# Antiparadox/Spartan-BN254

Hardware: AMD Instinct MI355X
Metric: msm_points_per_s (higher is better)
Workload: dtype u32; 1 GPU; synthetic BN254 G1 MSM, 2^20 uniform Fr scalars x distinct bases per GPU, inputs resident in HBM; steps_in_flight=6

## Files before the change

spartan-bn254_amd/csrc/glv_kernels.cuh:

```cuda
#pragma once
#include "msm_kernels.cuh"

namespace sbn {

namespace glv {
constexpr uint64_t A[2] = {0x8211bbeb7d4f1128ull, 0x6f4d8248eeb859fcull};
constexpr uint64_t B = 0x89d3256894d213e3ull;
constexpr uint64_t C[2] = {0x0be4e1541221250bull, 0x6f4d8248eeb859fdull};
constexpr uint64_t G1[3] = {0x5398fd0300ff6565ull, 0x4ccef014a773d2d2ull, 0x2ull};
constexpr uint64_t G2[2] = {0xd91d232ec7e0b3d7ull, 0x2ull};
constexpr uint64_t R[4] = {0x43e1f593f0000001ull, 0x2833e84879b97091ull, 0xb85045b68181585dull, 0x30644e72e131a029ull};
constexpr uint32_t BETA[8] = {0x607cfd48u, 0xe4bd44e5u, 0xbb966e3du, 0xc28f069fu, 0xe0acccb0u, 0x5e6dd9e7u, 0xe131a029u, 0x30644e72u};
}

template <int NA, int NB>
__device__ __forceinline__ void glv_mul(const uint64_t (&a)[NA], const uint64_t (&b)[NB], uint64_t (&out)[NA + NB]) {
#pragma unroll
  for (int i = 0; i < NA + NB; i++) out[i] = 0;
#pragma unroll
  for (int i = 0; i < NA; i++) {
    uint64_t carry = 0;
#pragma unroll
    for (int j = 0; j < NB; j++) {
      const uint64_t lo = a[i] * b[j], hi = __umul64hi(a[i], b[j]);
// ... 15 lines not shown
    for (int j = 0; j < NB && i + j < 4; j++) {
      const uint64_t lo = a[i] * b[j], hi = __umul64hi(a[i], b[j]);
      uint64_t s = out[i + j] + lo; uint64_t cy = s < lo ? 1 : 0;
      s += carry; cy += s < carry ? 1 : 0;
      out[i + j] = s; carry = hi + cy;
    }
    if (i + NB < 4) out[i + NB] = carry;
  }
}
__device__ __forceinline__ bool glv_diff_ge_r(const uint64_t (&x)[4], const uint64_t (&y)[4]) {
  uint64_t d[4], borrow = 0;
#pragma unroll
  for (int i = 0; i < 4; i++) { const uint64_t t = x[i] - y[i]; const uint64_t b1 = x[i] < y[i]; d[i] = t - borrow; borrow = b1 | (t < borrow); }
#pragma unroll
  for (int i = 3; i >= 0; i--) { if (d[i] != glv::R[i]) return d[i] > glv::R[i]; }
  return true;
}
__device__ __forceinline__ void u128_mul_lo(uint64_t a0, uint64_t a1, uint64_t b0, uint64_t b1, uint64_t& o0, uint64_t& o1) {
  o0 = a0 * b0; o1 = __umul64hi(a0, b0) + a0 * b1 + a1 * b0;
}
__device__ __forceinline__ void u128_add(uint64_t& x0, uint64_t& x1, uint64_t y0, uint64_t y1) { const uint64_t s = x0 + y0; x1 += y1 + (s < x0 ? 1 : 0); x0 = s; }
__device__ __forceinline__ void u128_sub(uint64_t& x0, uint64_t& x1, uint64_t y0, uint64_t y1) { const uint64_t b = x0 < y0 ? 1 : 0; x0 -= y0; x1 -= y1 + b; }

__device__ __forceinline__ void glv_split(const uint64_t (&k)[4], uint64_t (&k1)[2], uint64_t (&k2)[2]) {
  uint64_t p1[7], p2[6];
  glv_mul<4, 3>(k, glv::G1, p1);
  glv_mul<4, 2>(k, glv::G2, p2);
  uint64_t c1[2] = {p1[4], p1[5]}, c2[1] = {p2[4]};
  {
    uint64_t kc[4], cr[4];
    glv_mul_lo256<2>(k, glv::C, kc);
    const uint64_t c1v[4] = {c1[0], c1[1], 0, 0};
    glv_mul_lo256<4>(c1v, glv::R, cr);
    if (glv_diff_ge_r(kc, cr)) { if (++c1[0] == 0) ++c1[1]; }
  }
  {
    uint64_t kb[4], cr[4];
    const uint64_t bb[1] = {glv::B};
    glv_mul_lo256<1>(k, bb, kb);
    const uint64_t c2v[4] = {c2[0], 0, 0, 0};
    glv_mul_lo256<4>(c2v, glv::R, cr);
    if (glv_diff_ge_r(kb, cr)) ++c2[0];
  }
  uint64_t x0 = k[0], x1 = k[1], t0, t1;
  u128_mul_lo(c1[0], c1[1], glv::A[0], glv::A[1], t0, t1); u128_sub(x0, x1, t0, t1);
  u128_mul_lo(c2[0], 0, glv::B, 0, t0, t1); u128_sub(x0, x1, t0, t1);
  uint64_t y0, y1;
  u128_mul_lo(c1[0], c1[1], glv::B, 0, y0, y1);
  u128_mul_lo(c2[0], 0, glv::C[0], glv::C[1], t0, t1); u128_sub(y0, y1, t0, t1);
  if (y1 >> 63) { u128_add(x0, x1, glv::B, 0); u128_add(y0, y1, glv::C[0], glv::C[1]); }
  k1[0] = x0; k1[1] = x1; k2[0] = y0; k2[1] = y1;
}

__global__ void __launch_bounds__(256) k_glv_split(const uint32_t* __restrict__ scalars, size_t n, uint32_t* __restrict__ out, uint32_t* __restrict__ bad) {
  const size_t t = (size_t)blockIdx.x * blockDim.x + threadIdx.x;
  if (t >= n) return;
  const uint4 a = reinterpret_cast<const uint4*>(scalars + 8 * t)[0], b = reinterpret_cast<const uint4*>(scalars + 8 * t)[1];
  const uint32_t kk[8] = {a.x, a.y, a.z, a.w, b.x, b.y, b.z, b.w};
  uint64_t k1[2] = {0, 0}, k2[2] = {0, 0};
  if (!fe_is_canonical<FrP>(kk)) atomicAdd(bad, 1u);
  else {
    const uint64_t k[4] = {(uint64_t)a.x | ((uint64_t)a.y << 32), (uint64_t)a.z | ((uint64_t)a.w << 32), (uint64_t)b.x | ((uint64_t)b.y << 32), (uint64_t)b.z | ((uint64_t)b.w << 32)};
    glv_split(k, k1, k2);
  }
  uint4* o = reinterpret_cast<uint4*>(out);
  o[t] = make_uint4((uint32_t)k1[0], (uint32_t)(k1[0] >> 32), (uint32_t)k1[1], (uint32_t)(k1[1] >> 32));
  o[n + t] = make_uint4((uint32_t)k2[0], (uint32_t)(k2[0] >> 32), (uint32_t)k2[1], (uint32_t)(k2[1] >> 32));
}

__global__ void __launch_bounds__(256) k_glv_table(const uint32_t* __restrict__ pts, size_t npts, uint32_t* __restrict__ out) {
  const size_t j = (size_t)blockIdx.x * blockDim.x + threadIdx.x;
  if (j >= npts) return;
  const uint4* s = reinterpret_cast<const uint4*>(pts + 16 * j);
  uint4* d0 = reinterpret_cast<uint4*>(out + 16 * j);
  uint4* d1 = reinterpret_cast<uint4*>(out + 16 * (npts + j));
  const uint4 w0 = s[0], w1 = s[1], w2 = s[2], w3 = s[3];
  d0[0] = w0; d0[1] = w1; d0[2] = w2; d0[3] = w3;
  const Fq beta = fe_to_mont(fe_unpack<FqP>(glv::BETA));
  const Fq x = fe_load<FqP>(pts + 16 * j);
  fe_store<FqP>(out + 16 * (npts + j), fe_mul(x, beta));
  d1[2] = w2; d1[3] = w3;
}

}
```

spartan-bn254_amd/csrc/msm_host.hpp:

```cpp
#pragma once
static int ilog2_ceil(size_t n) { int l = 0; while (((size_t)1 << l) < n) l++; return l; }

static MsmShape make_shape(int c, int bits = 254) {
  MsmShape s; s.c = c; s.nb = 1 << (c - 1);
  int W = (bits + c - 1) / c;
  int tb = bits - (W - 1) * c;
  if (tb > c - 1) W += 1;
  s.W = W;
  return s;
}
static MsmShape choose_shape(size_t terms, bool shared_bucket_set, int cmax, size_t problems = 0, int chard = MSM_C_MAX) {
  const char* env = getenv("SBN_MSM_C");
  if (env && atoi(env) >= 7 && atoi(env) <= chard) return make_shape(atoi(env));
  if (cmax > chard) cmax = chard;
  if (problems && problems * terms <= 32768) {
    if (!shared_bucket_set && problems == 1 && terms >= 512 && terms <= 4096 && cmax >= 8) return make_shape(terms <= 512 ? 8 : 7);
    double bl = 1e300; int bcl = 7;
    for (int c = 7; c <= cmax; c++) {
      MsmShape s = make_shape(c);
      const int tb = 254 - (s.W - 1) * c;
      const double top = (double)terms / (double)(1u << (tb > 0 ? (tb < 20 ? tb : 20) : 0));
      const double load = (shared_bucket_set ? (double)terms * s.W / s.nb : (double)terms / s.nb) + top;
      if (load <= 6.0) return s;
      if (load < bl) { bl = load; bcl = c; }
    }
    return make_shape(bcl);
  }
  if (!shared_bucket_set && terms < ((size_t)1 << 20) && cmax >= 15) return make_shape(15);
  double best = 1e300; int bc = 7;
  for (int c = 7; c <= cmax; c++) {
    MsmShape s = make_shape(c);
    double sets = shared_bucket_set ? 1.0 : (double)s.W;
    const double per_bucket = (chard > MSM_C_MAX || (shared_bucket_set && problems >= 256)) ? 40.0 : 56.0;
    double cost = (double)terms * s.W * 10.0 + sets * s.nb * per_bucket;
    if (!shared_bucket_set && 254 - (s.W - 1) * c < c - 1) cost += (double)terms * 5.0;
    if (cost < best) { best = cost; bc = c; }
  }
  return make_shape(bc);
}

#define S2_FOR_EACH_C(X) X(13) X(14) X(15) X(16) X(17) X(18) X(19) X(20) X(21) X(22)
#define S2_GLV_FOR_EACH_C(X) X(13) X(14) X(15) X(16) X(17)
static bool sort2_set_lds() {
  bool ok = true;
  const int bytes = (int)s2_scatter_lds_bytes(S2_P_MAX);
  if (hipFuncSetAttribute((const void*)k_s2_place, hipFuncAttributeMaxDynamicSharedMemorySize, (int)s2_place_lds_bytes(S2_LO_LOG_MAX)) != hipSuccess) { (void)hipGetLastError(); ok = false; }
#define X(C) if (hipFuncSetAttribute((const void*)k_s2_scatter<C, S2_SPT>, hipFuncAttributeMaxDynamicSharedMemorySize, bytes) != hipSuccess) { (void)hipGetLastError(); ok = false; } \
             if (hipFuncSetAttribute((const void*)k_s2_scatter<C, S2_SPT_SMALL>, hipFuncAttributeMaxDynamicSharedMemorySize, bytes) != hipSuccess) { (void)hipGetLastError(); ok = false; }
  S2_FOR_EACH_C(X)
#undef X
  const int cnt_bytes = 24 * S2_P_MAX * 4;
#define X(C) if (hipFuncSetAttribute((const void*)k_s2_count<C, S2_SPT>, hipFuncAttributeMaxDynamicSharedMemorySize, cnt_bytes) != hipSuccess) { (void)hipGetLastError(); ok = false; } \
             if (hipFuncSetAttribute((const void*)k_s2_count<C, S2_SPT_SMALL>, hipFuncAttributeMaxDynamicSharedMemorySize, cnt_bytes) != hipSuccess) { (void)hipGetLastError(); ok = false; }
  S2_FOR_EACH_C(X)
#undef X
#define X(C) if (hipFuncSetAttribute((const void*)k_s2_count<C, S2_SPT, 4>, hipFuncAttributeMaxDynamicSharedMemorySize, cnt_bytes) != hipSuccess) { (void)hipGetLastError(); ok = false; } \
             if (hipFuncSetAttribute((const void*)k_s2_count<C, S2_SPT_SMALL, 4>, hipFuncAttributeMaxDynamicSharedMemorySize, cnt_bytes) != hipSuccess) { (void)hipGetLastError(); ok = false; } \
             if (hipFuncSetAttribute((const void*)k_s2_scatter<C, S2_SPT, 4>, hipFuncAttributeMaxDynamicSharedMemorySize, bytes) != hipSuccess) { (void)hipGetLastError(); ok = false; } \
             if (hipFuncSetAttribute((const void*)k_s2_scatter<C, S2_SPT_SMALL, 4>, hipFuncAttributeMaxDynamicSharedMemorySize, bytes) != hipSuccess) { (void)hipGetLastError(); ok = false; }
  S2_GLV_FOR_EACH_C(X)
#undef X
  return ok;
}
static bool sort2_applies(const sbn_ctx* c, int mode, size_t n, int cbits) {
  return mode == MODE_SINGLE && c->sort2_ok && c->sort2_min && n >= c->sort2_min && cbits >= S2_C_MIN && cbits <= S2_C_MAX;
}
static int sort2_run(sbn_ctx* c, const uint32_t* scalars, size_t n, const MsmShape& s, size_t estride, uint32_t* hist, uint32_t* offs, uint32_t* sorted, bool glv = false, size_t glv_gap = 0) {
  S2Geom g; g.n = n; g.c = s.c; g.W = s.W; g.half = n / 2; g.gap = glv ? glv_gap : 0;
  if (glv && (s.c < 13 || s.c > 17)) return fail(c, SBN_EINVAL, "two-level sort: no GLV instantiation for windows of %d bits", s.c);
  g.lo_log = std::max(s.c - 1 - 8, 8); if (g.lo_log > S2_LO_LOG_MAX) g.lo_log = S2_LO_LOG_MAX;
  if (const char* e = getenv("SBN_SORT2_LO")) { int v = atoi(e); if (v >= 4 && v <= S2_LO_LOG_MAX) g.lo_log = v; }
  if (s.c - 1 - g.lo_log < 0) g.lo_log = s.c - 1;
  while ((s.nb >> g.lo_log) > S2_P_MAX) g.lo_log++;
  if (g.lo_log > S2_LO_LOG_MAX) return fail(c, SBN_EINVAL, "two-level sort: window of %d bits is too wide", s.c);
  g.P = s.nb >> g.lo_log;
  const int LO = 1 << g.lo_log;
  int spt = (n <= ((size_t)1 << 21) && g.P <= 64) ? S2_SPT_SMALL : S2_SPT;
  if (const char* e = getenv("SBN_SORT2_SPT")) { const int v = atoi(e); if (v == S2_SPT || v == S2_SPT_SMALL) spt = v; }
  const size_t ch = (size_t)1024 * spt;
  g.K = (int)((n + ch - 1) / ch);
  const size_t WP = (size_t)g.W * g.P;
  const size_t max_sc = ((size_t)g.W * n) / S2_SUB + WP;
  int rc;
  if ((rc = ensure(c, c->s2_cnt, WP * g.K * 4))) return rc;
  if ((rc = ensure(c, c->s2_part, (3 * WP + 1) * 4))) return rc;
  if ((rc = ensure(c, c->s2_idx, (size_t)g.W * n * 4))) return rc;
  if ((rc = ensure(c, c->s2_lo, (size_t)g.W * n * 2))) return rc;
  if ((rc = ensure(c, c->blockhist, max_sc * LO * 4))) return rc;
  uint32_t* cntA = (uint32_t*)c->s2_cnt.p; uint32_t* part_cnt = (uint32_t*)c->s2_part.p; uint32_t* part_off = part_cnt + WP; uint32_t* sc_off = part_off + WP;
  uint32_t* tmp_idx = (uint32_t*)c->s2_idx.p; uint16_t* tmp_lo = (uint16_t*)c->s2_lo.p; uint32_t* bh = (uint32_t*)c->blockhist.p;
  const size_t lds_a = WP * 4, lds_c = s2_scatter_lds_bytes(g.P, spt);
  if (lds_a > (size_t)24 * S2_P_MAX * 4) return fail(c, SBN_EINVAL, "two-level sort: %zu level-1 counters do not fit the LDS granted to k_s2_count", WP);
  {
    ProfScope _ps(c, "k_s2_count");
    if (glv) switch (s.c) {
#define X(C) case C: if (spt == S2_SPT) hipLaunchKernelGGL((k_s2_count<C, S2_SPT, 4>), dim3(g.K), dim3(1024), lds_a, c->stream, scalars, g, cntA, c->d_bad); \
                     else hipLaunchKernelGGL((k_s2_count<C, S2_SPT_SMALL, 4>), dim3(g.K), dim3(1024), lds_a, c->stream, scalars, g, cntA, c->d_bad); break;
      S2_GLV_FOR_EACH_C(X)
#undef X
    } else switch (s.c) {
#define X(C) case C: if (spt == S2_SPT) hipLaunchKernelGGL((k_s2_count<C, S2_SPT>), dim3(g.K), dim3(1024), lds_a, c->stream, scalars, g, cntA, c->d_bad); \
                     else hipLaunchKernelGGL((k_s2_count<C, S2_SPT_SMALL>), dim3(g.K), dim3(1024), lds_a, c->stream, scalars, g, cntA, c->d_bad); break;
      S2_FOR_EACH_C(X)
#undef X
    }
  }
  LAUNCH(c, "k_s2_prefix", k_s2_prefix_k, (unsigned)WP, 256, cntA, g.K, part_cnt);
  LAUNCH(c, "k_s2_prefix", k_s2_prefix_hi, 1, 1024, (const uint32_t*)part_cnt, g.W, g.P, part_off, sc_off);
  {
    ProfScope _ps(c, "k_s2_scatter");
    if (glv) switch (s.c) {
#define X(C) case C: if (spt == S2_SPT) hipLaunchKernelGGL((k_s2_scatter<C, S2_SPT, 4>), dim3(g.K), dim3(1024), lds_c, c->stream, scalars, g, (const uint32_t*)cntA, (const uint32_t*)part_off, tmp_idx, tmp_lo); \
                     else hipLaunchKernelGGL((k_s2_scatter<C, S2_SPT_SMALL, 4>), dim3(g.K), dim3(1024), lds_c, c->stream, scalars, g, (const uint32_t*)cntA, (const uint32_t*)part_off, tmp_idx, tmp_lo); break;
      S2_GLV_FOR_EACH_C(X)
#undef X
    } else switch (s.c) {
#define X(C) case C: if (spt == S2_SPT) hipLaunchKernelGGL((k_s2_scatter<C, S2_SPT>), dim3(g.K), dim3(1024), lds_c, c->stream, scalars, g, (const uint32_t*)cntA, (const uint32_t*)part_off, tmp_idx, tmp_lo); \
                     else hipLaunchKernelGGL((k_s2_scatter<C, S2_SPT_SMALL>), dim3(g.K), dim3(1024), lds_c, c->stream, scalars, g, (const uint32_t*)cntA, (const uint32_t*)part_off, tmp_idx, tmp_lo); break;
      S2_FOR_EACH_C(X)
#undef X
    }
  }
  const unsigned l2 = s2_level2_blocks(max_sc);
  LAUNCH(c, "k_s2_hist", k_s2_hist, l2, 1024, (const uint16_t*)tmp_lo, g, (const uint32_t*)part_off, (const uint32_t*)part_cnt, (const uint32_t*)sc_off, bh);
  LAUNCH(c, "k_s2_prefix", k_s2_prefix2, (unsigned)WP, 1024, bh, g, (const uint32_t*)part_off, (const uint32_t*)sc_off, hist, offs);
  {
    ProfScope _ps(c, "k_s2_place");
    hipLaunchKernelGGL(k_s2_place, dim3(l2), dim3(1024), s2_place_lds_bytes(g.lo_log), c->stream,
                       (const uint16_t*)tmp_lo, (const uint32_t*)tmp_idx, g, (const uint32_t*)part_off, (const uint32_t*)part_cnt, (const uint32_t*)sc_off, (const uint32_t*)bh, (const uint32_t*)offs, sorted, estride);
  }
  LAUNCHCHK(c);
  return SBN_OK;
}

struct BucketJob {
  int mode; DigitArgs da; MsmShape s;
  size_t P;
  size_t threads;
  const uint32_t* points;
  const uint8_t* skip;
  bool glv;
  size_t glv_gap;
};

static int run_bucket_job(sbn_ctx* c, const BucketJob& J) {
  const MsmShape& s = J.s;
  const size_t NB = J.P * (size_t)s.nb;
  if (NB > 0xffffffffull) return fail(c, SBN_EINVAL, "bucket space too large");
  const size_t estride = J.da.estride;
  c->last_job[0] = (uint64_t)s.c; c->last_job[1] = (uint64_t)s.W; c->last_job[2] = (uint64_t)(J.P * estride); c->last_job[3] = (uint64_t)NB;
  size_t mean = estride / (size_t)s.nb + 1;
  uint32_t SEG = 32; while (SEG < 2 * mean && SEG < ACC_SEG_MAX) SEG <<= 1;
  if (NB < 262144) { const size_t total = J.P * estride; uint32_t cap = 32; while ((size_t)cap * 262144 < total && cap < ACC_SEG_MAX) cap <<= 1; if (SEG > cap) SEG = cap; }
  if (J.mode == MODE_SINGLE && J.da.n >= 512 && J.da.n <= 4096) SEG = 8;
  if (const char* es = getenv("SBN_MSM_SEG")) { int v = atoi(es); if (v >= 8 && v <= (int)ACC_SEG_MAX) SEG = (uint32_t)v; }
  int LPB = 1; if (J.mode == MODE_SINGLE && mean >= 48 && NB <= ((size_t)1 << 19)) LPB = 2;
  const size_t max_extra = J.P * estride / SEG + 1;
  const size_t max_big = std::min(NB, max_extra);
  int rc;
  if ((rc = ensure(c, c->hist, NB * 4))) return rc;
  if ((rc = ensure(c, c->offs, NB * 4))) return rc;
  if ((rc = ensure(c, c->sorted, J.P * estride * 4))) return rc;
  if ((rc = ensure(c, c->buckets, NB * 128 * (size_t)LPB))) return rc;
  if ((rc = ensure(c, c->acc_ctr, 64 + (ACC_SEG_MAX + 2) * 4))) return rc;
  if ((rc = ensure(c, c->extra_list, max_extra * sizeof(ExtraItem)))) return rc;
  if ((rc = ensure(c, c->extra_out, max_extra * 128))) return rc;
  if ((rc = ensure(c, c->big_list, max_big * sizeof(BigItem)))) return rc;
  int L = 1; while ((size_t)L * 64 * 2048 < NB && L < 16) L <<= 1;
  if (L < 4) L = 4;
  if (L > s.nb / 64) L = s.nb / 64;
  if (L < 1) L = 1;
  if (NB <= (size_t)64 * 16 * 1024) {
    double best = 1e300; int bl = L;
    for (int t = 1; t <= 32 && t * 64 <= std::max(s.nb, 64); t++) {
      const size_t waves = J.P * (size_t)((s.nb + 64 * t - 1) / (64 * t));
      const double cost = (double)((waves + 1023) / 1024) * (double)((2 * t - 1) + t * (LPB - 1) + 10);
      if (cost < best) { best = cost; bl = t; }
    }
    L = bl;
  }
  if (const char* el = getenv("SBN_RED_L")) { int v = atoi(el); if (v >= 1 && v <= 64) L = v; }
  const int chunks = (s.nb + 64 * L - 1) / (64 * L);
  if ((rc = ensure(c, c->red_a, J.P * chunks * 256))) return rc;
  if ((rc = ensure(c, c->red_b, J.P * ((chunks + 63) / 64) * 256))) return rc;
  if ((rc = ensure(c, c->wsum, J.P * 128))) return rc;

  uint32_t* hist = (uint32_t*)c->hist.p; uint32_t* offs = (uint32_t*)c->offs.p;
  uint32_t* sorted = (uint32_t*)c->sorted.p; uint32_t* buckets = (uint32_t*)c->buckets.p;
  AccCounters* ctr = (AccCounters*)c->acc_ctr.p;

  static_assert(sizeof(AccCounters) <= 64, "the size bins follow the counters at byte 64");
  HIPCHK(c, hipMemsetAsync(ctr, 0, 64 + (ACC_SEG_MAX + 2) * 4, c->stream));
  SortGeom g; memset(&g, 0, sizeof g);
  g.E = estride; g.estride = estride; g.nb = s.nb; g.mode = J.mode; g.ncol = J.da.n; g.tstride = J.da.tstride;
  g.RS = std::min(s.nb, c->sort_rs_max); g.logRS = 0; while ((1 << g.logRS) < g.RS) g.logRS++;
  g.R = s.nb / g.RS;
  { size_t want = (1024 + J.P * g.R - 1) / (J.P * g.R); size_t maxk = std::max<size_t>(1, estride / 4096); g.K = (int)std::max<size_t>(1, std::min(want, maxk)); }
  g.chunk = (estride + g.K - 1) / g.K;
  const uint8_t* skip = nullptr;
  const bool two_level = sort2_applies(c, J.mode, J.da.n, s.c) && !J.skip;
  if (s.c > MSM_C_MAX && !two_level) return fail(c, SBN_EINVAL, "window of %d bits needs the two-level sort", s.c);
  if (J.glv && !two_level) return fail(c, SBN_EINVAL, "GLV half-scalars need the two-level sort");
  if (two_level) {
    if ((rc = sort2_run(c, J.da.scalars, J.da.n, s, estride, hist, offs, sorted, J.glv, J.glv_gap))) return rc;
  } else {
  if (J.P > 65535 || g.R > 65535) return fail(c, SBN_EINVAL, "sort grid too large (P=%zu R=%d)", J.P, g.R);
  if ((rc = ensure(c, c->digits, J.P * estride * sizeof(dig_t)))) return rc;
  if ((rc = ensure(c, c->blockhist, J.P * (size_t)g.R * g.K * g.RS * 4))) return rc;
  dig_t* dig = (dig_t*)c->digits.p; uint32_t* bh = (uint32_t*)c->blockhist.p;
  const unsigned gd = (unsigned)((J.threads + 255) / 256);
  const size_t rows_lds = sort_rows_lds_bytes(s.nb);
  const bool fused_rows = J.mode == MODE_ROWS && c->sort_rows_ok && rows_lds <= 160 * 1024 && estride <= 8 * (size_t)SORT_SL;
  skip = fused_rows ? J.skip : nullptr;
  if (J.mode == MODE_SINGLE) LAUNCH(c, "k_digits_store", (k_digits_store<MODE_SINGLE>), gd, 256, J.da, s, dig, (const uint8_t*)nullptr);
  else LAUNCH(c, "k_digits_store", (k_digits_store<MODE_ROWS>), gd, 256, J.da, s, dig, skip);
  if (c->z_consumed && J.mode == MODE_ROWS) HIPCHK(c, hipEventRecord(c->z_consumed, c->stream));
  if (fused_rows) {
    ProfScope _ps(c, "k_sort_rows");
    hipLaunchKernelGGL(k_sort_rows, dim3((unsigned)J.P), dim3(1024), rows_lds, c->stream, (const dig_t*)dig, g, hist, offs, sorted, skip);
  } else {
    {
      ProfScope _ps(c, "k_hist_lds");
      hipLaunchKernelGGL(k_hist_lds, dim3(g.K, g.R, (unsigned)J.P), dim3(1024), (size_t)g.RS * 4, c->stream, (const dig_t*)dig, g, bh);
    }
    LAUNCH(c, "k_block_prefix", k_block_prefix, (unsigned)((NB + 255) / 256), 256, bh, g, NB, hist);
    LAUNCH(c, "k_scan", k_scan, (unsigned)J.P, 1024, hist, offs, s.nb);
    {
      ProfScope _ps(c, "k_scatter_lds");
      hipLaunchKernelGGL(k_scatter_lds, dim3(g.K, g.R, (unsigned)J.P), dim3(1024), (size_t)g.RS * 4, c->stream, (const dig_t*)dig, g, (const uint32_t*)bh, (const uint32_t*)offs, sorted);
    }
  }
  }
  if ((rc = ensure(c, c->perm, NB * 4))) return rc;
  uint32_t* size_bins = (uint32_t*)((uint8_t*)c->acc_ctr.p + 64);
  LAUNCH(c, "k_size_sort", k_size_hist, (unsigned)((NB + 1023) / 1024), 1024, hist, NB, SEG, size_bins);
  LAUNCH(c, "k_size_sort", k_size_scan, 1, 64, size_bins, SEG);
  LAUNCH(c, "k_size_sort", k_size_scatter, (unsigned)((NB + 1023) / 1024), 1024, hist, NB, SEG, size_bins, (uint32_t*)c->perm.p);
  const unsigned agrid = (unsigned)((NB * (size_t)LPB + 255) / 256);
#define ACC_FIRST_ARGS J.points, NB, s.nb, estride, SEG, hist, offs, sorted, (const uint32_t*)c->perm.p, buckets, ctr, (ExtraItem*)c->extra_list.p, (BigItem*)c->big_list.p
  if (LPB == 1) LAUNCH(c, "k_acc_first", k_acc_first<1>, agrid, 256, ACC_FIRST_ARGS);
  else LAUNCH(c, "k_acc_first", k_acc_first<2>, agrid, 256, ACC_FIRST_ARGS);
#undef ACC_FIRST_ARGS
  LAUNCH(c, "k_acc_extra", k_acc_extra, 2048, 256, J.points, s.nb, estride, SEG, hist, offs, sorted, ctr, (const ExtraItem*)c->extra_list.p, (uint32_t*)c->extra_out.p);
  LAUNCH(c, "k_acc_merge", k_acc_merge, 4096, 64, ctr, (const BigItem*)c->big_list.p, (const uint32_t*)c->extra_out.p, buckets, LPB);
  const bool red_quad = J.P * (size_t)chunks <= 2048;
  LAUNCH(c, "k_reduce_l1", k_reduce_l1, (unsigned)(J.P * chunks), 64, buckets, L, s.nb, (uint32_t*)c->red_a.p, skip, chunks, LPB);
  uint32_t* in = (uint32_t*)c->red_a.p; uint32_t* outb = (uint32_t*)c->red_b.p;
  int G = chunks, k64 = 1;
  for (;;) {
    int Gout = (G + 63) / 64;
    int final = (Gout == 1);
    if (red_quad) LAUNCH(c, "k_reduce_combine", k_reduce_combine_quad, (unsigned)(J.P * Gout), 256, in, G, Gout, k64, L, final, final ? (uint32_t*)c->wsum.p : outb);
    else LAUNCH(c, "k_reduce_combine", k_reduce_combine, (unsigned)(J.P * Gout), 64, in, G, Gout, k64, L, final, final ? (uint32_t*)c->wsum.p : outb);
    if (final) break;
    std::swap(in, outb); G = Gout; k64 += 1;
  }
  LAUNCHCHK(c);
  return SBN_OK;
}

static std::mutex g_bases_tables_mu;

static double single_msm_cost(size_t terms, const MsmShape& s, int bits) {
  double cost = (double)terms * s.W * 10.0 + (double)s.W * s.nb * 40.0;
  if (bits - (s.W - 1) * s.c < s.c - 1) cost += (double)terms * 5.0;
  return cost;
}
static MsmShape glv_shape(size_t n) {
  if (const char* env = getenv("SBN_MSM_C")) { const int v = atoi(env); if (v >= 13 && v <= 17) return make_shape(v, 127); }
  MsmShape best = make_shape(16, 127);
  for (int cc = 13; cc <= 17; cc++) { const MsmShape s = make_shape(cc, 127); if (single_msm_cost(2 * n, s, 127) < single_msm_cost(2 * n, best, 127)) best = s; }
  return best;
}
static bool glv_applies(const sbn_ctx* c, const sbn_bases* b, size_t n, const MsmShape& plain) {
  if (!b || c->msm_glv == 0 || (c->msm_glv < 0 && getenv("SBN_MSM_C"))) return false;
  const size_t npts = b->n + (b->has_h ? 1 : 0);
  if (2 * npts > 0x7fffffffull || !sort2_applies(c, MODE_SINGLE, 2 * n, S2_C_MIN)) return false;
  if (c->msm_glv == 1) return true;
  return single_msm_cost(2 * n, glv_shape(n), 127) * 1.04 < single_msm_cost(n, plain, 254);
}
static int bases_glv_table(sbn_ctx* c, const sbn_bases* b, const uint32_t** out) {
  std::lock_guard<std::mutex> tg(g_bases_tables_mu);
  if (b->d_glv) { *out = (const uint32_t*)b->d_glv; return SBN_OK; }
  const size_t npts = b->n + (b->has_h ? 1 : 0);
  void* tab = nullptr;
  hipError_t e = hipMalloc(&tab, 2 * npts * 64);
  if (e != hipSuccess) { (void)hipGetLastError(); return fail(c, SBN_ENOMEM, "hipMalloc GLV table (%zu B): %s", 2 * npts * 64, hipGetErrorString(e)); }
  LAUNCH(c, "k_glv_table", k_glv_table, (unsigned)((npts + 255) / 256), 256, (const uint32_t*)b->d_pts, npts, (uint32_t*)tab);
  hipError_t le = hipGetLastError();
  hipError_t se = hipStreamSynchronize(c->stream);
  if (le != hipSuccess || se != hipSuccess) { hipFree(tab); return fail(c, SBN_EHIP, "GLV table build: %s", hipGetErrorString(le != hipSuccess ? le : se)); }
  b->d_glv = tab;
  *out = (const uint32_t*)tab;
  return SBN_OK;
}

static int msm_device(sbn_ctx* c, const uint32_t* d_scal, const uint32_t* d_bases, size_t n, uint8_t out_xy[64], int* out_is_inf, const sbn_bases* b = nullptr) {
  if (n == 0) { memset(out_xy, 0, 64); if (out_is_inf) *out_is_inf = 1; return SBN_OK; }
  if (n > 0x7fffffffull) return fail(c, SBN_EINVAL, "msm: n=%zu exceeds 2^31-1", n);
  BucketJob J; memset(&J, 0, sizeof J);
  J.mode = MODE_SINGLE;
  {
    int cm = 1; while ((1 << cm) < c->sort_rs_max) cm++;
    const bool s2 = sort2_applies(c, MODE_SINGLE, n, S2_C_MIN);
    J.s = choose_shape(n, false, s2 ? S2_C_MAX : cm + 1, 1, s2 ? S2_C_MAX : MSM_C_MAX);
  }
  J.P = (size_t)J.s.W; J.threads = n; J.points = d_bases;
  J.da.scalars = d_scal; J.da.n = n; J.da.estride = n; J.da.bad = c->d_bad;
  const bool glv = glv_applies(c, b, n, J.s);
  int rc;
  if (glv) {
    const uint32_t* tab;
    if ((rc = bases_glv_table(c, b, &tab))) return rc;
    if ((rc = ensure(c, c->glv_scal, 2 * n * 16))) return rc;
    J.s = glv_shape(n); J.P = (size_t)J.s.W; J.threads = 2 * n; J.points = tab;
    J.da.scalars = (const uint32_t*)c->glv_scal.p; J.da.n = 2 * n; J.da.estride = 2 * n;
    J.glv = true; J.glv_gap = b->n + (b->has_h ? 1 : 0) - n;
  }
  if ((rc = ensure_pin(c, std::max<size_t>(4096, J.P * 128)))) return rc;
  if ((rc = input_check_begin(c))) return rc;
  if (glv) LAUNCH(c, "k_glv_split", k_glv_split, (unsigned)((n + 255) / 256), 256, d_scal, n, (uint32_t*)c->glv_scal.p, c->d_bad);
  if ((rc = run_bucket_job(c, J))) return rc;
  HIPCHK(c, hipMemcpyAsync(c->pin, c->wsum.p, J.P * 128, hipMemcpyDeviceToHost, c->stream));
  if ((rc = input_check_fetch(c))) return rc;
  HIPCHK(c, hipStreamSynchronize(c->stream));
  if (c->prof) prof_drain(c);
  if ((rc = input_check_end(c))) return rc;
  std::vector<sbn_host::Pt> S((size_t)J.s.W);
  for (int w = 0; w < J.s.W; w++) S[(size_t)w] = sbn_host::pt_from_device(((const sbn_host::Pt*)c->pin)[w]);
  sbn_host::Pt total = sbn_host::combine_windows(S.data(), J.s.W, J.s.c);
  sbn_host::to_affine_bytes(total, out_xy, out_is_inf);
  return SBN_OK;
}

static int bases_window_table(sbn_ctx* c, const sbn_bases* b, const MsmShape& s, const uint32_t** out) {
  std::lock_guard<std::mutex> tg(g_bases_tables_mu);
  auto it = b->tables.find(s.c);
  if (it != b->tables.end()) { *out = (const uint32_t*)it->second; return SBN_OK; }
  const size_t npts = b->n + (b->has_h ? 1 : 0);
  const size_t tot = npts * (size_t)s.W;
  int rc;
  if ((rc = ensure(c, c->gen_tmp, tot * 128))) return rc;
  void* tab = nullptr;
  hipError_t e = hipMalloc(&tab, tot * 64);
  if (e != hipSuccess) return fail(c, SBN_ENOMEM, "hipMalloc window table (%zu B): %s", tot * 64, hipGetErrorString(e));
  LAUNCH(c, "k_window_table", k_window_table, (unsigned)((npts + 63) / 64), 64, (const uint32_t*)b->d_pts, npts, s.c, s.W, (uint32_t*)c->gen_tmp.p);
  LAUNCH(c, "k_xyzz_to_affine", k_xyzz_to_affine, (unsigned)((tot + 63) / 64), 64, (const uint32_t*)c->gen_tmp.p, (uint32_t*)tab, (uint32_t*)nullptr, (uint8_t*)nullptr, tot);
  LAUNCHCHK(c);
  HIPCHK(c, hipStreamSynchronize(c->stream));
  b->tables[s.c] = tab;
  *out = (const uint32_t*)tab;
  return SBN_OK;
}

static int bases_build_comb(sbn_ctx* c, sbn_bases* b, size_t max_bytes) {
  const size_t npts = b->n + (b->has_h ? 1 : 0);
  if (npts == 0) return fail(c, SBN_EINVAL, "precompute: empty generator set");
  int cc = 0; size_t bytes = 0;
  for (int t = COMB_C_MAX; t >= 7; t--) {
    const MsmShape s = make_shape(t);
    const size_t need = npts * (size_t)s.W * (size_t)s.nb * 64;
    if (need <= max_bytes) { cc = t; bytes = need; break; }
  }
  if (!cc) return fail(c, SBN_EINVAL, "precompute: even the c = 7 table (%zu B) exceeds the budget of %zu B", npts * (size_t)make_shape(7).W * 64 * 64, max_bytes);
  {
    std::lock_guard<std::mutex> tg(g_bases_tables_mu);
    if (b->d_comb && b->comb_c == cc) return SBN_OK;
  }
  const MsmShape s = make_shape(cc);
  int rc; const uint32_t* wtab;
  if ((rc = bases_window_table(c, b, s, &wtab))) return rc;
  std::lock_guard<std::mutex> tg(g_bases_tables_mu);
  if (b->d_comb) { HIPCHK(c, hipStreamSynchronize(c->stream)); hipFree(b->d_comb); b->d_comb = nullptr; b->comb_c = 0; }
  void* tab = nullptr;
// ... 205 lines not shown
```

spartan-bn254_amd/csrc/sort2_kernels.cuh:

```cuda
#pragma once
#include "msm_kernels.cuh"
#include <utility>

namespace sbn {

constexpr int S2_LO_LOG_MAX = 11, S2_LO_MAX = 1 << S2_LO_LOG_MAX;
constexpr int S2_P_MAX = 1024;
constexpr int S2_SPT = 8, S2_CH = 1024 * S2_SPT;
constexpr int S2_SPT_SMALL = 2;
constexpr int S2_C_MIN = 13, S2_C_MAX = 22;
struct S2Geom {
  size_t n;
  int c, W, P;
  int lo_log;
  int K;
  size_t half, gap;
};

template <int C, int SW = 8> struct S2Shape {
  static constexpr int BITS = SW == 8 ? 254 : 127;
  static constexpr int W0 = (BITS + C - 1) / C;
  static constexpr int W = W0 + ((BITS - (W0 - 1) * C) > C - 1 ? 1 : 0);
};
typedef uint32_t s2_u32x8 __attribute__((ext_vector_type(8)));
template <int C, int w> __device__ __forceinline__ int s2_digit(const s2_u32x8 k, uint32_t& carry) {
  constexpr int bit = w * C, limb = bit >> 5, sh = bit & 31;
  uint64_t x = 0;
  if constexpr (limb < 8) x = k[limb];
  if constexpr (limb + 1 < 8) x |= (uint64_t)k[limb + 1] << 32;
  const uint32_t raw = (uint32_t)(x >> sh) & ((1u << C) - 1u);
  const uint32_t v = raw + carry;
  if (v >= (1u << (C - 1))) { carry = 1; return (int)v - (1 << C); }
  carry = 0;
  return (int)v;
}
template <int SW = 8> __device__ __forceinline__ s2_u32x8 s2_load_scalar(const uint32_t* __restrict__ scalars, size_t t) {
  const uint4* p = reinterpret_cast<const uint4*>(scalars + (size_t)SW * t);
  const uint4 a = p[0], b = SW == 8 ? p[1] : make_uint4(0u, 0u, 0u, 0u);
  s2_u32x8 k; k[0] = a.x; k[1] = a.y; k[2] = a.z; k[3] = a.w; k[4] = b.x; k[5] = b.y; k[6] = b.z; k[7] = b.w;
  return k;
}
__device__ __forceinline__ bool s2_is_canonical(const s2_u32x8 k) { uint32_t kk[8]; for (int i = 0; i < 8; i++) kk[i] = k[i]; return fe_is_canonical<FrP>(kk); }

extern __shared__ uint32_t s2_lds[];

template <int C, int... Ws>
__device__ __forceinline__ void s2_count_scalar(const s2_u32x8 kk, int P, int lo_log, std::integer_sequence<int, Ws...>) {
  uint32_t carry = 0;
  auto one = [&](auto wc) {
    constexpr int w = decltype(wc)::value;
    const int d = s2_digit<C, w>(kk, carry);
    if (d != 0) atomicAdd(&s2_lds[w * P + (((d < 0 ? -d : d) - 1) >> lo_log)], 1u);
  };
  (one(std::integral_constant<int, Ws>{}), ...);
}
template <int C, int SPT, int SW = 8>
__global__ void __launch_bounds__(1024) k_s2_count(const uint32_t* __restrict__ scalars, S2Geom g, uint32_t* __restrict__ cntA, uint32_t* __restrict__ bad) {
  constexpr int W = S2Shape<C, SW>::W; constexpr int CH = 1024 * SPT;
  const int k = blockIdx.x, P = g.P;
  for (int j = threadIdx.x; j < W * P; j += 1024) s2_lds[j] = 0;
  __syncthreads();
  for (int i = 0; i < SPT; i++) {
    const size_t t = (size_t)k * CH + (size_t)i * 1024 + threadIdx.x;
    if (t >= g.n) break;
    const s2_u32x8 kk = s2_load_scalar<SW>(scalars, t);
    if (SW == 8 && !s2_is_canonical(kk)) atomicAdd(bad, 1u);
    s2_count_scalar<C>(kk, P, g.lo_log, std::make_integer_sequence<int, W>{});
  }
  __syncthreads();
  for (int j = threadIdx.x; j < W * P; j += 1024) cntA[(size_t)j * g.K + k] = s2_lds[j];
}

__device__ __forceinline__ uint32_t s2_block_scan(uint32_t v, uint32_t* tmp , uint32_t* total) {
  const int lane = threadIdx.x & 63, wv = threadIdx.x >> 6, nw = (blockDim.x + 63) >> 6;
  uint32_t inc = v;
#pragma unroll
  for (int d = 1; d < 64; d <<= 1) { const uint32_t o = __shfl_up(inc, d); if (lane >= d) inc += o; }
  if (lane == 63) tmp[wv] = inc;
  __syncthreads();
  if (threadIdx.x == 0) { uint32_t run = 0; for (int i = 0; i < nw; i++) { const uint32_t x = tmp[i]; tmp[i] = run; run += x; } tmp[16] = run; }
  __syncthreads();
  const uint32_t r = inc - v + tmp[wv];
  *total = tmp[16];
  __syncthreads();
  return r;
}
__global__ void __launch_bounds__(256) k_s2_prefix_k(uint32_t* __restrict__ cntA, int K, uint32_t* __restrict__ part_cnt) {
  __shared__ uint32_t tmp[17];
  uint32_t* row = cntA + (size_t)blockIdx.x * K;
  const int per = (K + 255) / 256, b0 = threadIdx.x * per;
  uint32_t sum = 0;
  for (int i = 0; i < per; i++) if (b0 + i < K) sum += row[b0 + i];
  uint32_t total; uint32_t run = s2_block_scan(sum, tmp, &total);
  for (int i = 0; i < per; i++) if (b0 + i < K) { const uint32_t v = row[b0 + i]; row[b0 + i] = run; run += v; }
  if (threadIdx.x == 0) part_cnt[blockIdx.x] = total;
}
constexpr uint32_t S2_SUB = 16384;
__global__ void __launch_bounds__(1024) k_s2_prefix_hi(const uint32_t* __restrict__ part_cnt, int W, int P, uint32_t* __restrict__ part_off, uint32_t* __restrict__ sc_off) {
  __shared__ uint32_t tmp[17];
  __shared__ uint32_t wstart[32];
  const int n = W * P, per = (n + 1023) / 1024, i0 = (int)threadIdx.x * per, i1 = (i0 + per < n) ? i0 + per : n;
  uint32_t sv = 0, sk = 0;
  for (int i = i0; i < i1; i++) { const uint32_t v = part_cnt[i]; sv += v; sk += (v + S2_SUB - 1) / S2_SUB; }
  uint32_t tv, tk;
  uint32_t rv = s2_block_scan(sv, tmp, &tv), rk = s2_block_scan(sk, tmp, &tk);
  for (int i = i0; i < i1; i++) { const uint32_t v = part_cnt[i]; part_off[i] = rv; sc_off[i] = rk; rv += v; rk += (v + S2_SUB - 1) / S2_SUB; }
  if (threadIdx.x == 0) sc_off[(size_t)n] = tk;
  __syncthreads();
  if ((int)threadIdx.x < W) wstart[threadIdx.x] = part_off[(size_t)threadIdx.x * P];
  __syncthreads();
  for (int i = i0; i < i1; i++) part_off[i] -= wstart[i / P];
}

__host__ __device__ inline size_t s2_scatter_lds_bytes(int P, int spt = S2_SPT) { return ((size_t)3 * P + 32) * 4 + (size_t)1024 * spt * 8; }
struct S2ScatterArgs {
  const uint32_t* cntA; const uint32_t* part_off; uint32_t* tmp_idx; uint16_t* tmp_lo;
  size_t n, half, gap; int P, K, k, lo_log;
};
template <int C, int w, int SPT>
__device__ __forceinline__ void s2_scatter_window(const s2_u32x8 (&kk)[SPT], uint32_t (&carry)[SPT], const S2ScatterArgs& a) {
  constexpr int CH = 1024 * SPT;
  const int P = a.P, tid = threadIdx.x;
  uint32_t* cnt = s2_lds; uint32_t* base = cnt + P; uint32_t* gdelta = base + P; uint32_t* tmp = gdelta + P;
  uint32_t* stage_idx = tmp + 32;
  uint16_t* stage_lo = reinterpret_cast<uint16_t*>(stage_idx + CH); uint16_t* stage_hi = stage_lo + CH;
  for (int j = tid; j < P; j += 1024) cnt[j] = 0;
  __syncthreads();
  int d[SPT]; uint32_t rank[SPT];
#pragma unroll
  for (int i = 0; i < SPT; i++) {
    const int dd = s2_digit<C, w>(kk[i], carry[i]);
    d[i] = dd; rank[i] = 0;
    if (dd != 0) rank[i] = atomicAdd(&cnt[((dd < 0 ? -dd : dd) - 1) >> a.lo_log], 1u);
  }
  __syncthreads();
  uint32_t total;
  {
    const uint32_t v = tid < P ? cnt[tid] : 0;
    const uint32_t r = s2_block_scan(v, tmp, &total);
    if (tid < P) { base[tid] = r; gdelta[tid] = a.part_off[(size_t)w * P + tid] + a.cntA[((size_t)w * P + tid) * a.K + a.k] - r; }
  }
  __syncthreads();
  const size_t t0 = (size_t)a.k * CH + tid;
#pragma unroll
  for (int i = 0; i < SPT; i++) {
    if (d[i] == 0) continue;
    const uint32_t b = (uint32_t)((d[i] < 0 ? -d[i] : d[i]) - 1), hi = b >> a.lo_log;
    const uint32_t pos = base[hi] + rank[i];
    size_t e = t0 + (size_t)i * 1024;
    if (a.gap && e >= a.half) e += a.gap;
    stage_idx[pos] = (uint32_t)e | (d[i] < 0 ? 0x80000000u : 0u);
    stage_lo[pos] = (uint16_t)(b & ((1u << a.lo_log) - 1u)); stage_hi[pos] = (uint16_t)hi;
  }
  __syncthreads();
  uint32_t* oi = a.tmp_idx + (size_t)w * a.n; uint16_t* ol = a.tmp_lo + (size_t)w * a.n;
  for (uint32_t j = tid; j < total; j += 1024) {
    const uint32_t pos = j + gdelta[stage_hi[j]];
    oi[pos] = stage_idx[j]; ol[pos] = stage_lo[j];
  }
  __syncthreads();
}
template <int C, int SPT, int... Ws>
__device__ __forceinline__ void s2_scatter_windows(const s2_u32x8 (&kk)[SPT], uint32_t (&carry)[SPT], const S2ScatterArgs& a, std::integer_sequence<int, Ws...>) {
  (s2_scatter_window<C, Ws, SPT>(kk, carry, a), ...);
}
template <int C, int SPT, int SW = 8>
__global__ void __launch_bounds__(1024) k_s2_scatter(const uint32_t* __restrict__ scalars, S2Geom g, const uint32_t* __restrict__ cntA ,
                                                     const uint32_t* __restrict__ part_off, uint32_t* __restrict__ tmp_idx, uint16_t* __restrict__ tmp_lo) {
  S2ScatterArgs a; a.cntA = cntA; a.part_off = part_off; a.tmp_idx = tmp_idx; a.tmp_lo = tmp_lo; a.n = g.n; a.P = g.P; a.K = g.K; a.k = blockIdx.x; a.lo_log = g.lo_log;
  a.half = g.half; a.gap = SW == 8 ? 0 : g.gap;
  s2_u32x8 kk[SPT]; uint32_t carry[SPT];
#pragma unroll
  for (int i = 0; i < SPT; i++) {
    const size_t t = (size_t)blockIdx.x * (1024 * SPT) + (size_t)i * 1024 + threadIdx.x;
    carry[i] = 0;
    kk[i] = t < g.n ? s2_load_scalar<SW>(scalars, t) : (s2_u32x8)(0u);
  }
  s2_scatter_windows<C, SPT>(kk, carry, a, std::make_integer_sequence<int, S2Shape<C, SW>::W>{});
}

__device__ __forceinline__ bool s2_decode(const S2Geom& g, const uint32_t* __restrict__ sc_off, int& q, uint32_t& sidx, uint32_t& k2) {
  const uint32_t Lid = blockIdx.x, xcd = Lid & 7u, slot = Lid >> 3;
  sidx = (slot >> 4) * 128u + xcd * 16u + (slot & 15u);
  const int WP = g.W * g.P;
  if (sidx >= sc_off[WP]) return false;
  int lo = 0, hi = WP;
  while (hi - lo > 1) { const int mid = (lo + hi) >> 1; if (sc_off[mid] <= sidx) lo = mid; else hi = mid; }
  q = lo; k2 = sidx - sc_off[q];
  return true;
}
__host__ __device__ inline uint32_t s2_level2_blocks(size_t max_subchunks) { return (uint32_t)(((max_subchunks + 127) / 128) * 128); }
__device__ __forceinline__ void s2_range(const S2Geom& g, const uint32_t* __restrict__ part_off, const uint32_t* __restrict__ part_cnt, int q, uint32_t k2, size_t& e0, size_t& e1) {
  const uint32_t start = part_off[q], cn = part_cnt[q];
  uint32_t a = k2 * S2_SUB, b = a + S2_SUB; if (a > cn) a = cn; if (b > cn) b = cn;
  const size_t w = (size_t)(q / g.P);
  e0 = w * g.n + start + a; e1 = w * g.n + start + b;
}
__global__ void __launch_bounds__(1024) k_s2_hist(const uint16_t* __restrict__ tmp_lo, S2Geom g, const uint32_t* __restrict__ part_off, const uint32_t* __restrict__ part_cnt, const uint32_t* __restrict__ sc_off, uint32_t* __restrict__ blockhist) {
  __shared__ uint32_t h[S2_LO_MAX];
  int q; uint32_t sidx, k2; if (!s2_decode(g, sc_off, q, sidx, k2)) return;
  const int LO = 1 << g.lo_log;
  for (int j = threadIdx.x; j < LO; j += 1024) h[j] = 0;
  __syncthreads();
  size_t e0, e1; s2_range(g, part_off, part_cnt, q, k2, e0, e1);
  for (size_t e = e0 + threadIdx.x; e < e1; e += 1024) atomicAdd(&h[tmp_lo[e]], 1u);
  __syncthreads();
  uint32_t* o = blockhist + (size_t)sidx * LO;
  for (int j = threadIdx.x; j < LO; j += 1024) o[j] = h[j];
}
__global__ void __launch_bounds__(1024) k_s2_prefix2(uint32_t* __restrict__ blockhist, S2Geom g, const uint32_t* __restrict__ part_off, const uint32_t* __restrict__ sc_off, uint32_t* __restrict__ hist, uint32_t* __restrict__ offs) {
  __shared__ uint32_t tmp[17];
  const int q = blockIdx.x, LO = 1 << g.lo_log, w = q / g.P, hi = q - w * g.P;
  const uint32_t s0 = sc_off[q], nk = sc_off[q + 1] - s0;
  const int j0 = 2 * threadIdx.x;
  uint32_t r0 = 0, r1 = 0;
  if (j0 < LO) {
    uint2* col = reinterpret_cast<uint2*>(blockhist + (size_t)s0 * LO + j0);
    for (uint32_t k = 0; k < nk; k++) { uint2* pq = col + (size_t)k * (LO / 2); const uint2 v = *pq; *pq = make_uint2(r0, r1); r0 += v.x; r1 += v.y; }
  }
  uint32_t total; const uint32_t r = s2_block_scan(r0 + r1, tmp, &total);
  if (j0 < LO) {
    const size_t b = ((size_t)w * g.P + hi) * LO + j0;
    hist[b] = r0; hist[b + 1] = r1;
// ... 58 lines not shown
```

Baseline: 702.6 million points/s.

## Fuse GLV scalar split into sort count kernel and tune accumulation lanes

Removes the separate k_glv_split launch and performs the GLV decomposition inside k_s2_count, writing interleaved half-scalar records and counting digits directly from registers. The scatter's index mapping changes from a half/gap layout to an interleaved even/odd layout to match. The accumulation lanes-per-bucket choice is extended to 1–4 via a cost model with new k_acc_first instantiations. The reduce-level choice also gains a combine-level cost term. This saves one launch and one pass over the scalars, but makes the count kernel heavier, which may lower its occupancy.

```diff
diff --git a/spartan-bn254_amd/csrc/glv_kernels.cuh b/spartan-bn254_amd/csrc/glv_kernels.cuh
--- a/spartan-bn254_amd/csrc/glv_kernels.cuh
+++ b/spartan-bn254_amd/csrc/glv_kernels.cuh
@@ -91,20 +91,17 @@
   k1[0] = x0; k1[1] = x1; k2[0] = y0; k2[1] = y1;
 }
 
-__global__ void __launch_bounds__(256) k_glv_split(const uint32_t* __restrict__ scalars, size_t n, uint32_t* __restrict__ out, uint32_t* __restrict__ bad) {
-  const size_t t = (size_t)blockIdx.x * blockDim.x + threadIdx.x;
-  if (t >= n) return;
-  const uint4 a = reinterpret_cast<const uint4*>(scalars + 8 * t)[0], b = reinterpret_cast<const uint4*>(scalars + 8 * t)[1];
+__device__ __forceinline__ bool glv_split_records(const uint4 a, const uint4 b, uint4& r1, uint4& r2) {
   const uint32_t kk[8] = {a.x, a.y, a.z, a.w, b.x, b.y, b.z, b.w};
   uint64_t k1[2] = {0, 0}, k2[2] = {0, 0};
-  if (!fe_is_canonical<FrP>(kk)) atomicAdd(bad, 1u);
-  else {
+  const bool ok = fe_is_canonical<FrP>(kk);
+  if (ok) {
     const uint64_t k[4] = {(uint64_t)a.x | ((uint64_t)a.y << 32), (uint64_t)a.z | ((uint64_t)a.w << 32), (uint64_t)b.x | ((uint64_t)b.y << 32), (uint64_t)b.z | ((uint64_t)b.w << 32)};
     glv_split(k, k1, k2);
   }
-  uint4* o = reinterpret_cast<uint4*>(out);
-  o[t] = make_uint4((uint32_t)k1[0], (uint32_t)(k1[0] >> 32), (uint32_t)k1[1], (uint32_t)(k1[1] >> 32));
-  o[n + t] = make_uint4((uint32_t)k2[0], (uint32_t)(k2[0] >> 32), (uint32_t)k2[1], (uint32_t)(k2[1] >> 32));
+  r1 = make_uint4((uint32_t)k1[0], (uint32_t)(k1[0] >> 32), (uint32_t)k1[1], (uint32_t)(k1[1] >> 32));
+  r2 = make_uint4((uint32_t)k2[0], (uint32_t)(k2[0] >> 32), (uint32_t)k2[1], (uint32_t)(k2[1] >> 32));
+  return ok;
 }
 
 __global__ void __launch_bounds__(256) k_glv_table(const uint32_t* __restrict__ pts, size_t npts, uint32_t* __restrict__ out) {
diff --git a/spartan-bn254_amd/csrc/msm_host.hpp b/spartan-bn254_amd/csrc/msm_host.hpp
--- a/spartan-bn254_amd/csrc/msm_host.hpp
+++ b/spartan-bn254_amd/csrc/msm_host.hpp
@@ -65,8 +65,9 @@
 static bool sort2_applies(const sbn_ctx* c, int mode, size_t n, int cbits) {
   return mode == MODE_SINGLE && c->sort2_ok && c->sort2_min && n >= c->sort2_min && cbits >= S2_C_MIN && cbits <= S2_C_MAX;
 }
-static int sort2_run(sbn_ctx* c, const uint32_t* scalars, size_t n, const MsmShape& s, size_t estride, uint32_t* hist, uint32_t* offs, uint32_t* sorted, bool glv = false, size_t glv_gap = 0) {
+static int sort2_run(sbn_ctx* c, const uint32_t* scalars, size_t n, const MsmShape& s, size_t estride, uint32_t* hist, uint32_t* offs, uint32_t* sorted, bool glv = false, size_t glv_gap = 0, const uint32_t* glv_src = nullptr) {
   S2Geom g; g.n = n; g.c = s.c; g.W = s.W; g.half = n / 2; g.gap = glv ? glv_gap : 0;
+  if (glv && (!glv_src || (n & 1))) return fail(c, SBN_EINVAL, "two-level sort: GLV records without their scalars");
   if (glv && (s.c < 13 || s.c > 17)) return fail(c, SBN_EINVAL, "two-level sort: no GLV instantiation for windows of %d bits", s.c);
   g.lo_log = std::max(s.c - 1 - 8, 8); if (g.lo_log > S2_LO_LOG_MAX) g.lo_log = S2_LO_LOG_MAX;
   if (const char* e = getenv("SBN_SORT2_LO")) { int v = atoi(e); if (v >= 4 && v <= S2_LO_LOG_MAX) g.lo_log = v; }
@@ -94,13 +95,13 @@
   {
     ProfScope _ps(c, "k_s2_count");
     if (glv) switch (s.c) {
-#define X(C) case C: if (spt == S2_SPT) hipLaunchKernelGGL((k_s2_count<C, S2_SPT, 4>), dim3(g.K), dim3(1024), lds_a, c->stream, scalars, g, cntA, c->d_bad); \
-                     else hipLaunchKernelGGL((k_s2_count<C, S2_SPT_SMALL, 4>), dim3(g.K), dim3(1024), lds_a, c->stream, scalars, g, cntA, c->d_bad); break;
+#define X(C) case C: if (spt == S2_SPT) hipLaunchKernelGGL((k_s2_count<C, S2_SPT, 4>), dim3(g.K), dim3(1024), lds_a, c->stream, glv_src, g, cntA, c->d_bad, const_cast<uint32_t*>(scalars)); \
+                     else hipLaunchKernelGGL((k_s2_count<C, S2_SPT_SMALL, 4>), dim3(g.K), dim3(1024), lds_a, c->stream, glv_src, g, cntA, c->d_bad, const_cast<uint32_t*>(scalars)); break;
       S2_GLV_FOR_EACH_C(X)
 #undef X
     } else switch (s.c) {
-#define X(C) case C: if (spt == S2_SPT) hipLaunchKernelGGL((k_s2_count<C, S2_SPT>), dim3(g.K), dim3(1024), lds_a, c->stream, scalars, g, cntA, c->d_bad); \
-                     else hipLaunchKernelGGL((k_s2_count<C, S2_SPT_SMALL>), dim3(g.K), dim3(1024), lds_a, c->stream, scalars, g, cntA, c->d_bad); break;
+#define X(C) case C: if (spt == S2_SPT) hipLaunchKernelGGL((k_s2_count<C, S2_SPT>), dim3(g.K), dim3(1024), lds_a, c->stream, scalars, g, cntA, c->d_bad, (uint32_t*)nullptr); \
+                     else hipLaunchKernelGGL((k_s2_count<C, S2_SPT_SMALL>), dim3(g.K), dim3(1024), lds_a, c->stream, scalars, g, cntA, c->d_bad, (uint32_t*)nullptr); break;
       S2_FOR_EACH_C(X)
 #undef X
     }
@@ -133,6 +134,11 @@
   return SBN_OK;
 }
 
+constexpr int ACC_G_MAX = 4;
+constexpr size_t ACC_RESIDENT_BLOCKS = 768;
+constexpr double ACC_LANE_FIXED = 2.0;
+constexpr double RED_COMBINE_LEVEL_COST = 18.0;
+
 struct BucketJob {
   int mode; DigitArgs da; MsmShape s;
   size_t P;
@@ -141,6 +147,7 @@
   const uint8_t* skip;
   bool glv;
   size_t glv_gap;
+  const uint32_t* glv_src;
 };
 
 static int run_bucket_job(sbn_ctx* c, const BucketJob& J) {
@@ -154,7 +161,18 @@
   if (NB < 262144) { const size_t total = J.P * estride; uint32_t cap = 32; while ((size_t)cap * 262144 < total && cap < ACC_SEG_MAX) cap <<= 1; if (SEG > cap) SEG = cap; }
   if (J.mode == MODE_SINGLE && J.da.n >= 512 && J.da.n <= 4096) SEG = 8;
   if (const char* es = getenv("SBN_MSM_SEG")) { int v = atoi(es); if (v >= 8 && v <= (int)ACC_SEG_MAX) SEG = (uint32_t)v; }
-  int LPB = 1; if (J.mode == MODE_SINGLE && mean >= 48 && NB <= ((size_t)1 << 19)) LPB = 2;
+  int LPB = 1;
+  if (J.mode == MODE_SINGLE && mean >= 48 && NB <= ((size_t)1 << 19)) {
+    double best = 1e300;
+    for (int t = 2; t <= ACC_G_MAX; t++) {
+      const size_t blocks = (NB * (size_t)t + 255) / 256;
+      const double rounds = (double)((blocks + ACC_RESIDENT_BLOCKS - 1) / ACC_RESIDENT_BLOCKS);
+      const double fold = (double)(t - 1) * (double)NB * 14.0 / ((double)ACC_RESIDENT_BLOCKS * 256.0 * 10.0);
+      const double cost = rounds * ((double)mean / t + ACC_LANE_FIXED) + fold;
+      if (cost < best) { best = cost; LPB = t; }
+    }
+  }
+  if (J.mode == MODE_SINGLE) if (const char* eg = getenv("SBN_ACC_G")) { const int v = atoi(eg); if (v >= 1 && v <= ACC_G_MAX) LPB = v; }
   const size_t max_extra = J.P * estride / SEG + 1;
   const size_t max_big = std::min(NB, max_extra);
   int rc;
@@ -173,8 +191,10 @@
   if (NB <= (size_t)64 * 16 * 1024) {
     double best = 1e300; int bl = L;
     for (int t = 1; t <= 32 && t * 64 <= std::max(s.nb, 64); t++) {
-      const size_t waves = J.P * (size_t)((s.nb + 64 * t - 1) / (64 * t));
-      const double cost = (double)((waves + 1023) / 1024) * (double)((2 * t - 1) + t * (LPB - 1) + 10);
+      const size_t per = (size_t)((s.nb + 64 * t - 1) / (64 * t));
+      const size_t waves = J.P * per;
+      int levels = 1; for (size_t gch = (per + 63) / 64; gch > 1; gch = (gch + 63) / 64) levels++;
+      const double cost = (double)((waves + 1023) / 1024) * (double)((2 * t - 1) + t * (LPB - 1) + 10) + levels * RED_COMBINE_LEVEL_COST;
       if (cost < best) { best = cost; bl = t; }
     }
     L = bl;
@@ -202,7 +222,7 @@
   if (s.c > MSM_C_MAX && !two_level) return fail(c, SBN_EINVAL, "window of %d bits needs the two-level sort", s.c);
   if (J.glv && !two_level) return fail(c, SBN_EINVAL, "GLV half-scalars need the two-level sort");
   if (two_level) {
-    if ((rc = sort2_run(c, J.da.scalars, J.da.n, s, estride, hist, offs, sorted, J.glv, J.glv_gap))) return rc;
+    if ((rc = sort2_run(c, J.da.scalars, J.da.n, s, estride, hist, offs, sorted, J.glv, J.glv_gap, J.glv_src))) return rc;
   } else {
   if (J.P > 65535 || g.R > 65535) return fail(c, SBN_EINVAL, "sort grid too large (P=%zu R=%d)", J.P, g.R);
   if ((rc = ensure(c, c->digits, J.P * estride * sizeof(dig_t)))) return rc;
@@ -238,8 +258,12 @@
   LAUNCH(c, "k_size_sort", k_size_scatter, (unsigned)((NB + 1023) / 1024), 1024, hist, NB, SEG, size_bins, (uint32_t*)c->perm.p);
   const unsigned agrid = (unsigned)((NB * (size_t)LPB + 255) / 256);
 #define ACC_FIRST_ARGS J.points, NB, s.nb, estride, SEG, hist, offs, sorted, (const uint32_t*)c->perm.p, buckets, ctr, (ExtraItem*)c->extra_list.p, (BigItem*)c->big_list.p
-  if (LPB == 1) LAUNCH(c, "k_acc_first", k_acc_first<1>, agrid, 256, ACC_FIRST_ARGS);
-  else LAUNCH(c, "k_acc_first", k_acc_first<2>, agrid, 256, ACC_FIRST_ARGS);
+  switch (LPB) {
+    case 1: LAUNCH(c, "k_acc_first", k_acc_first<1>, agrid, 256, ACC_FIRST_ARGS); break;
+    case 2: LAUNCH(c, "k_acc_first", k_acc_first<2>, agrid, 256, ACC_FIRST_ARGS); break;
+    case 3: LAUNCH(c, "k_acc_first", k_acc_first<3>, agrid, 256, ACC_FIRST_ARGS); break;
+    default: LAUNCH(c, "k_acc_first", k_acc_first<4>, agrid, 256, ACC_FIRST_ARGS); break;
+  }
 #undef ACC_FIRST_ARGS
   LAUNCH(c, "k_acc_extra", k_acc_extra, 2048, 256, J.points, s.nb, estride, SEG, hist, offs, sorted, ctr, (const ExtraItem*)c->extra_list.p, (uint32_t*)c->extra_out.p);
   LAUNCH(c, "k_acc_merge", k_acc_merge, 4096, 64, ctr, (const BigItem*)c->big_list.p, (const uint32_t*)c->extra_out.p, buckets, LPB);
@@ -315,11 +339,10 @@
     if ((rc = ensure(c, c->glv_scal, 2 * n * 16))) return rc;
     J.s = glv_shape(n); J.P = (size_t)J.s.W; J.threads = 2 * n; J.points = tab;
     J.da.scalars = (const uint32_t*)c->glv_scal.p; J.da.n = 2 * n; J.da.estride = 2 * n;
-    J.glv = true; J.glv_gap = b->n + (b->has_h ? 1 : 0) - n;
+    J.glv = true; J.glv_gap = b->n + (b->has_h ? 1 : 0) - n; J.glv_src = d_scal;
   }
   if ((rc = ensure_pin(c, std::max<size_t>(4096, J.P * 128)))) return rc;
   if ((rc = input_check_begin(c))) return rc;
-  if (glv) LAUNCH(c, "k_glv_split", k_glv_split, (unsigned)((n + 255) / 256), 256, d_scal, n, (uint32_t*)c->glv_scal.p, c->d_bad);
   if ((rc = run_bucket_job(c, J))) return rc;
   HIPCHK(c, hipMemcpyAsync(c->pin, c->wsum.p, J.P * 128, hipMemcpyDeviceToHost, c->stream));
   if ((rc = input_check_fetch(c))) return rc;
diff --git a/spartan-bn254_amd/csrc/sort2_kernels.cuh b/spartan-bn254_amd/csrc/sort2_kernels.cuh
--- a/spartan-bn254_amd/csrc/sort2_kernels.cuh
+++ b/spartan-bn254_amd/csrc/sort2_kernels.cuh
@@ -1,5 +1,6 @@
 #pragma once
 #include "msm_kernels.cuh"
+#include "glv_kernels.cuh"
 #include <utility>
 
 namespace sbn {
@@ -55,17 +56,35 @@
   (one(std::integral_constant<int, Ws>{}), ...);
 }
 template <int C, int SPT, int SW = 8>
-__global__ void __launch_bounds__(1024) k_s2_count(const uint32_t* __restrict__ scalars, S2Geom g, uint32_t* __restrict__ cntA, uint32_t* __restrict__ bad) {
+__global__ void __launch_bounds__(1024) k_s2_count(const uint32_t* __restrict__ scalars, S2Geom g, uint32_t* __restrict__ cntA, uint32_t* __restrict__ bad, uint32_t* __restrict__ glv_out) {
   constexpr int W = S2Shape<C, SW>::W; constexpr int CH = 1024 * SPT;
   const int k = blockIdx.x, P = g.P;
   for (int j = threadIdx.x; j < W * P; j += 1024) s2_lds[j] = 0;
   __syncthreads();
-  for (int i = 0; i < SPT; i++) {
-    const size_t t = (size_t)k * CH + (size_t)i * 1024 + threadIdx.x;
-    if (t >= g.n) break;
-    const s2_u32x8 kk = s2_load_scalar<SW>(scalars, t);
-    if (SW == 8 && !s2_is_canonical(kk)) atomicAdd(bad, 1u);
-    s2_count_scalar<C>(kk, P, g.lo_log, std::make_integer_sequence<int, W>{});
+  if constexpr (SW == 4) {
+    static_assert(SPT % 2 == 0, "a block owns whole scalars");
+    for (int i = 0; i < SPT / 2; i++) {
+      const size_t t = (size_t)k * (CH / 2) + (size_t)i * 1024 + threadIdx.x;
+      if (t >= g.half) break;
+      const uint4* p = reinterpret_cast<const uint4*>(scalars + 8 * t);
+      uint4 r1, r2;
+      if (!glv_split_records(p[0], p[1], r1, r2)) atomicAdd(bad, 1u);
+      uint4* o = reinterpret_cast<uint4*>(glv_out + 8 * t);
+      o[0] = r1; o[1] = r2;
+      s2_u32x8 kk = (s2_u32x8)(0u);
+      kk[0] = r1.x; kk[1] = r1.y; kk[2] = r1.z; kk[3] = r1.w;
+      s2_count_scalar<C>(kk, P, g.lo_log, std::make_integer_sequence<int, W>{});
+      kk[0] = r2.x; kk[1] = r2.y; kk[2] = r2.z; kk[3] = r2.w;
+      s2_count_scalar<C>(kk, P, g.lo_log, std::make_integer_sequence<int, W>{});
+    }
+  } else {
+    for (int i = 0; i < SPT; i++) {
+      const size_t t = (size_t)k * CH + (size_t)i * 1024 + threadIdx.x;
+      if (t >= g.n) break;
+      const s2_u32x8 kk = s2_load_scalar<SW>(scalars, t);
+      if (!s2_is_canonical(kk)) atomicAdd(bad, 1u);
+      s2_count_scalar<C>(kk, P, g.lo_log, std::make_integer_sequence<int, W>{});
+    }
   }
   __syncthreads();
   for (int j = threadIdx.x; j < W * P; j += 1024) cntA[(size_t)j * g.K + k] = s2_lds[j];
@@ -115,7 +134,7 @@
 __host__ __device__ inline size_t s2_scatter_lds_bytes(int P, int spt = S2_SPT) { return ((size_t)3 * P + 32) * 4 + (size_t)1024 * spt * 8; }
 struct S2ScatterArgs {
   const uint32_t* cntA; const uint32_t* part_off; uint32_t* tmp_idx; uint16_t* tmp_lo;
-  size_t n, half, gap; int P, K, k, lo_log;
+  size_t n, phi; int P, K, k, lo_log, glv;
 };
 template <int C, int w, int SPT>
 __device__ __forceinline__ void s2_scatter_window(const s2_u32x8 (&kk)[SPT], uint32_t (&carry)[SPT], const S2ScatterArgs& a) {
@@ -148,7 +167,7 @@
     const uint32_t b = (uint32_t)((d[i] < 0 ? -d[i] : d[i]) - 1), hi = b >> a.lo_log;
     const uint32_t pos = base[hi] + rank[i];
     size_t e = t0 + (size_t)i * 1024;
-    if (a.gap && e >= a.half) e += a.gap;
+    if (a.glv) e = (e >> 1) + ((e & 1) ? a.phi : 0);
     stage_idx[pos] = (uint32_t)e | (d[i] < 0 ? 0x80000000u : 0u);
     stage_lo[pos] = (uint16_t)(b & ((1u << a.lo_log) - 1u)); stage_hi[pos] = (uint16_t)hi;
   }
@@ -168,7 +187,7 @@
 __global__ void __launch_bounds__(1024) k_s2_scatter(const uint32_t* __restrict__ scalars, S2Geom g, const uint32_t* __restrict__ cntA ,
                                                      const uint32_t* __restrict__ part_off, uint32_t* __restrict__ tmp_idx, uint16_t* __restrict__ tmp_lo) {
   S2ScatterArgs a; a.cntA = cntA; a.part_off = part_off; a.tmp_idx = tmp_idx; a.tmp_lo = tmp_lo; a.n = g.n; a.P = g.P; a.K = g.K; a.k = blockIdx.x; a.lo_log = g.lo_log;
-  a.half = g.half; a.gap = SW == 8 ? 0 : g.gap;
+  a.glv = SW == 4; a.phi = g.half + g.gap;
   s2_u32x8 kk[SPT]; uint32_t carry[SPT];
 #pragma unroll
   for (int i = 0; i < SPT; i++) {
```

Result: slower. 679.0 million points/s (-3.4%).
